# Roboy/gym-roboy

Hardware: AMD Instinct MI355X
Metric: env-steps/sec, MsjRobot (3-DOF/8-tendon) batched rollout (higher is better)
Workload: dtype f32

## Files before the change

### gym_roboy_amd/csrc/msj_kernels.hpp

```cpp
#pragma once
#include "rtc_compat.hpp"
#include "msj_math.hpp"
#include "philox.hpp"
#include "env_common.hpp"

#if defined(RB_JIT_TABLE)
namespace rbk { __device__ constexpr rb::MsjConst<float, 8> BAKED = RB_JIT_TABLE; }
#else
#include "msj_baked.hpp"
#endif

namespace rbk {

using rbe::EnvParams;
using rbe::GoalBox;
using rbe::goal_value;
using rbe::mul_then_add;

constexpr int NT8 = 8;
constexpr int RS = rb::MsjModel<float, 8>::RS;
using Const8 = rb::MsjConst<float, NT8>;
constexpr int NTX = 16;
using ConstX = rb::MsjConst<float, NTX>;

// ... 11 lines not shown

template <int KEEP>
struct SpSplit {
    const float *reg;
    const float *col;
    int stride;
    __device__ __forceinline__ float operator()(int k) const { return k < KEEP ? reg[k] : col[(k - KEEP) * stride]; }
};

struct Scale8 { float v[NT8]; };

template <int INTEG, int BLOCK, int UNROLL, bool BK = false>
__global__ void __launch_bounds__(BLOCK)
msj_step_env_per_lane(const Const8 c_arg, float *__restrict__ q, float *__restrict__ qd,
                      uint32_t *__restrict__ feas, const float *__restrict__ act, const Scale8 us, long n, long cnt) {
    const Const8 &c = robot_consts<BK>(c_arg);
    const long i = long(blockIdx.x) * BLOCK + threadIdx.x;
    if (i >= cnt) return;
    float qq[3], vv[3], sp[NT8];
    const float4 a0 = reinterpret_cast<const float4 *>(act)[2 * i];
    const float4 a1 = reinterpret_cast<const float4 *>(act)[2 * i + 1];
#pragma unroll
    for (int j = 0; j < 3; ++j) { qq[j] = q[j * n + i]; vv[j] = qd[j * n + i]; }
    const float a[NT8] = {a0.x, a0.y, a0.z, a0.w, a1.x, a1.y, a1.z, a1.w};
#pragma unroll
    for (int k = 0; k < NT8; ++k) sp[k] = a[k] * us.v[k];
    bool ok;
    if (UNROLL >= NT8) {
        ok = rb::MsjModel<float, NT8>::template step_sp<INTEG, UNROLL>(c, qq, vv, rb::SpArray<float, NT8>{sp});
    } else {
        __shared__ float lds_sp[NT8][BLOCK];
#pragma unroll
        for (int k = 0; k < NT8; ++k) lds_sp[k][threadIdx.x] = sp[k];
        ok = rb::MsjModel<float, NT8>::template step_sp<INTEG, UNROLL>(c, qq, vv, SpLds{&lds_sp[0][threadIdx.x], BLOCK});
    }
#pragma unroll
    for (int j = 0; j < 3; ++j) { q[j * n + i] = qq[j]; qd[j * n + i] = vv[j]; }
    feas[i] = ok ? 1u : 0u;
}




__device__ __forceinline__ __amdgpu_buffer_rsrc_t wg_rsrc(const void *base, int bytes) {
    return __builtin_amdgcn_make_buffer_rsrc(const_cast<void *>(base), 0, bytes, 0x00020000);
}

template <int INTEG, int BLOCK, bool BK = false>
__global__ void __launch_bounds__(BLOCK)
msj_step_env_per_lane_rs(const Const8 c_arg, float *__restrict__ q, float *__restrict__ qd,
                         uint32_t *__restrict__ feas, const float *__restrict__ act, const Scale8 us, long n, long cnt) {
    const Const8 &c = robot_consts<BK>(c_arg);
    const long env0 = long(blockIdx.x) * BLOCK;
    const long left = cnt - env0;
    const int live = int(left < BLOCK ? left : BLOCK);
    const int le = int(threadIdx.x);
    if (le >= live) return;
    const int off = le * 4;
    float qq[3], vv[3], u[NT8];
    const __amdgpu_buffer_rsrc_t ra = wg_rsrc(act + env0 * NT8, live * NT8 * 4);
    typedef float f4 __attribute__((ext_vector_type(4)));
    const f4 a0 = __builtin_bit_cast(f4, __builtin_amdgcn_raw_buffer_load_b128(ra, off * NT8, 0, 0));
    const f4 a1 = __builtin_bit_cast(f4, __builtin_amdgcn_raw_buffer_load_b128(ra, off * NT8 + 16, 0, 0));
#pragma unroll
    for (int j = 0; j < 3; ++j) {
        qq[j] = __uint_as_float(__builtin_amdgcn_raw_buffer_load_b32(wg_rsrc(q + j * n + env0, live * 4), off, 0, 0));
        vv[j] = __uint_as_float(__builtin_amdgcn_raw_buffer_load_b32(wg_rsrc(qd + j * n + env0, live * 4), off, 0, 0));
    }
    const float a[NT8] = {a0.x, a0.y, a0.z, a0.w, a1.x, a1.y, a1.z, a1.w};
#pragma unroll
    for (int k = 0; k < NT8; ++k) u[k] = a[k] * us.v[k];
    constexpr int KEEP = NT8 - 2;
    __shared__ float lds_u[NT8 - KEEP][BLOCK];
#pragma unroll
    for (int k = KEEP; k < NT8; ++k) lds_u[k - KEEP][le] = u[k];
    const bool ok = rb::MsjModel<float, NT8>::template step_rs_paired<INTEG>(c, qq, vv, SpSplit<KEEP>{u, &lds_u[0][le], BLOCK});
#pragma unroll
    for (int j = 0; j < 3; ++j) {
        __builtin_amdgcn_raw_buffer_store_b32(__float_as_uint(qq[j]), wg_rsrc(q + j * n + env0, live * 4), off, 0, 0);
        __builtin_amdgcn_raw_buffer_store_b32(__float_as_uint(vv[j]), wg_rsrc(qd + j * n + env0, live * 4), off, 0, 0);
    }
    __builtin_amdgcn_raw_buffer_store_b32(ok ? 1u : 0u, wg_rsrc(feas + env0, live * 4), off, 0, 0);
}


struct PairMap { int a[4], d[4]; };
struct Scale4 { float v[4]; };

template <int CTRL>
__device__ __forceinline__ float rbk_dpp(float v) {
    return __int_as_float(__builtin_amdgcn_update_dpp(0, __float_as_int(v), CTRL, 0xF, 0xF, true));
}

template <int MIRROR>
struct AccelMirrorHalf {
    const Const8 &c;
    const float *u;
    __device__ __forceinline__ void operator()(const float q[3], const float qd[3], float qdd[3]) const {
        using M = rb::MsjModel<float, NT8>;
        const M::Frame f = M::frame(q, qd);
        float tx, ty, tz;
        M::half_torque(c, f, u, tx, ty, tz);
        M::template mirror_combine<MIRROR>(tx, ty, tz, rbk_dpp<0xB1>(tx), rbk_dpp<0xB1>(ty), rbk_dpp<0xB1>(tz));
        M::rigid_body(c, f, qd, tx, ty, tz, qdd);
    }
};

template <int INTEG, int BLOCK, int MIRROR, bool BK = false>
__global__ void __launch_bounds__(BLOCK)
msj_step_mirror_pairs(const Const8 c_arg, const PairMap pm, float *__restrict__ q, float *__restrict__ qd,
                      uint32_t *__restrict__ feas, const float *__restrict__ act, const Scale4 us, long n, long cnt) {
    const Const8 &c = robot_consts<BK>(c_arg);
    const long env0 = long(blockIdx.x) * (BLOCK / 2);
    const long left = cnt - env0;
    const int live = int(left < BLOCK / 2 ? left : BLOCK / 2);
    const int le = int(threadIdx.x >> 1);
    if (le >= live) return;
    const bool odd = (threadIdx.x & 1) != 0;
    const int off = le * 4, oddi = int(threadIdx.x & 1);
    float qq[3], vv[3], u[4];
    const __amdgpu_buffer_rsrc_t ra = wg_rsrc(act + env0 * NT8, live * NT8 * 4);
#pragma unroll
    for (int k = 0; k < 4; ++k) u[k] = __uint_as_float(__builtin_amdgcn_raw_buffer_load_b32(ra, off * NT8 + pm.a[k] + oddi * pm.d[k], 0, 0)) * us.v[k];
#pragma unroll
    for (int j = 0; j < 3; ++j) {
        qq[j] = __uint_as_float(__builtin_amdgcn_raw_buffer_load_b32(wg_rsrc(q + j * n + env0, live * 4), off, 0, 0));
        vv[j] = __uint_as_float(__builtin_amdgcn_raw_buffer_load_b32(wg_rsrc(qd + j * n + env0, live * 4), off, 0, 0));
    }
    constexpr int F0 = MIRROR == 0 ? 0 : 1, F1 = 2;
    const uint32_t flip = odd ? 0x80000000u : 0u;
    qq[F0] = __uint_as_float(__float_as_uint(qq[F0]) ^ flip); vv[F0] = __uint_as_float(__float_as_uint(vv[F0]) ^ flip);
    qq[F1] = __uint_as_float(__float_as_uint(qq[F1]) ^ flip); vv[F1] = __uint_as_float(__float_as_uint(vv[F1]) ^ flip);
    const bool ok = rb::MsjModel<float, NT8>::template integrate_acc<INTEG>(c, qq, vv, AccelMirrorHalf<MIRROR>{c, u});
    const int soff = odd ? 0x7fffff00 : le * 4;
#pragma unroll
    for (int j = 0; j < 3; ++j) {
        __builtin_amdgcn_raw_buffer_store_b32(__float_as_uint(qq[j]), wg_rsrc(q + j * n + env0, live * 4), soff, 0, 0);
        __builtin_amdgcn_raw_buffer_store_b32(__float_as_uint(vv[j]), wg_rsrc(qd + j * n + env0, live * 4), soff, 0, 0);
    }
    __builtin_amdgcn_raw_buffer_store_b32(ok ? 1u : 0u, wg_rsrc(feas + env0, live * 4), soff, 0, 0);
}


template <int INTEG, int BLOCK, int UNROLL, bool BK = false>
__global__ void __launch_bounds__(BLOCK)
msj_rollout_fused(const Const8 c_arg, float *__restrict__ q, float *__restrict__ qd, uint32_t *__restrict__ feas,
                  const float *__restrict__ act_ring, int ring, int n_steps, const Scale8 us, long n) {
    const Const8 &c = robot_consts<BK>(c_arg);
    const long i = long(blockIdx.x) * BLOCK + threadIdx.x;
    if (i >= n) return;
    float qq[3], vv[3];
#pragma unroll
    for (int j = 0; j < 3; ++j) { qq[j] = q[j * n + i]; vv[j] = qd[j * n + i]; }
    bool ok = true;
    const float4 *rec = reinterpret_cast<const float4 *>(act_ring) + 2 * i;
    float4 a0 = rec[0], a1 = rec[1];
    __shared__ float lds_sp[UNROLL >= NT8 ? 1 : NT8][BLOCK];
    int slab = 0;
    for (int t = 0; t < n_steps; ++t) {
        const float a[NT8] = {a0.x, a0.y, a0.z, a0.w, a1.x, a1.y, a1.z, a1.w};
        float sp[NT8];
#pragma unroll
        for (int k = 0; k < NT8; ++k) sp[k] = a[k] * us.v[k];
        if (t + 1 < n_steps) {
            slab = slab + 1 == ring ? 0 : slab + 1;
            const float4 *nx = rec + long(slab) * 2 * n;
// ... 244 lines not shown
```

### gym_roboy_amd/csrc/msj_math.hpp

```cpp
#pragma once
#include "rtc_compat.hpp"

#if defined(__HIPCC__)
#define RB_HD __host__ __device__ __forceinline__
#else
#define RB_HD inline
#endif


namespace rb {

template <typename T> struct Fast;
template <> struct Fast<double> {
    static RB_HD void sincos(double x, double &s, double &c) { s = ::sin(x); c = ::cos(x); }
    static RB_HD double exp(double x) { return ::exp(x); }
    static RB_HD double exp2(double x) { return ::exp2(x); }
    static RB_HD double rsqrt(double x) { return 1.0 / ::sqrt(x); }
    static RB_HD double rcp(double x) { return 1.0 / x; }
};
template <> struct Fast<float> {
    static RB_HD void sincos(float x, float &s, float &c) {
#if defined(__HIP_DEVICE_COMPILE__)
        s = __sinf(x); c = __cosf(x);
#else
// ... 412 lines not shown
            }
            rigid_body(c, f, qd, tx, ty, tz, qdd);
        }
    };

    struct Routing { T d2, mx, my, mz; };
    static RB_HD Routing routing(const Frame &f, const MsjTendon<T> &t) {
        const T ax = f.r00 * t.A[0] + f.r10 * t.A[1] + f.r20 * t.A[2];
        const T ay = f.r01 * t.A[0] + f.r11 * t.A[1] + f.r21 * t.A[2];
        const T az = f.r02 * t.A[0] + f.r12 * t.A[1] + f.r22 * t.A[2];
        Routing r;
        r.d2 = ax * t.B2[0] + (ay * t.B2[1] + (az * t.B2[2] + t.ab2));
        r.mx = ay * t.Bv[2] - az * t.Bv[1];
        r.my = az * t.Bv[0] - ax * t.Bv[2];
        r.mz = ax * t.Bv[1] - ay * t.Bv[0];
        return r;
    }
    struct Strain { T v, es, fl, pe; };
    static RB_HD Strain strain(const C &c, const Frame &f, const MsjTendon<T> &t, const Routing &r, T inv) {
        Strain s;
        s.v = (f.wx * r.mx + f.wy * r.my + f.wz * r.mz) * inv;
        s.es = (r.d2 * inv) * t.il0s + t.elcs;
        s.fl = Fast<T>::exp2(-(s.es * s.es));
        s.pe = Fast<T>::exp2(c.pe_k2s * s.es);
        return s;
    }
    struct Hill { T afn, rden; };
    static RB_HD Hill hill(const C &c, const Strain &s, T u) {
        const T act = tclamp(c.kps * s.es - u, T(0), T(1));
        const T vp = tmax(s.v, T(0)), p = tclamp(s.v + T(1), T(0), T(1));
        const T num = c.fv_c1l * vp + p;
        const T den = c.fv_c2l * vp + (c.fv_c2s * p + c.fv_k);
        Hill h;
        h.rden = Fast<T>::rcp(den);
        h.afn = (act * s.fl) * num;
        return h;
    }
    static RB_HD void torque(const C &c, const MsjTendon<T> &t, const Routing &r, T inv, const Strain &s, const Hill &h,
                             T &tx, T &ty, T &tz) {
        const T fpe = tmax(s.pe * c.inv_pe_den - c.inv_pe_den, T(0));
        const T Fs = (t.fmaxv * inv) * (h.afn * h.rden + fpe);
        tx -= Fs * r.mx; ty -= Fs * r.my; tz -= Fs * r.mz;
    }
    static RB_HD void pin() {
#if defined(__HIP_DEVICE_COMPILE__)
        __builtin_amdgcn_sched_barrier(0);
#endif
    }
    static RB_HD void tendon_pair(const C &c, const Frame &f, const MsjTendon<T> &ta, const MsjTendon<T> &tb, T ua, T ub,
                                  T &tx, T &ty, T &tz) {
        const Routing ra = routing(f, ta);
        pin();
        const T ia = Fast<T>::rsqrt(ra.d2);
        const Routing rb_ = routing(f, tb);
        pin();
        const T ib = Fast<T>::rsqrt(rb_.d2);
        const Strain sa = strain(c, f, ta, ra, ia);
        pin();
        const Hill ha = hill(c, sa, ua);
        const Strain sb = strain(c, f, tb, rb_, ib);
        pin();
        torque(c, ta, ra, ia, sa, ha, tx, ty, tz);
        const Hill hb = hill(c, sb, ub);
        pin();
        torque(c, tb, rb_, ib, sb, hb, tx, ty, tz);
        pin();
    }
    template <typename SP>
    struct AccelPaired {
        const C &c;
        const SP &sp;
        RB_HD void operator()(const T q[3], const T qd[3], T qdd[3]) const {
            static_assert(NT % 2 == 0, "tendons in pairs");
            const Frame f = frame(q, qd);
            T tx = T(0), ty = T(0), tz = T(0);
#pragma unroll
            for (int k = 0; k < NT; k += 2) {
                const T ua = sp(k), ub = sp(k + 1);
                tendon_pair(c, f, c.ten[k], c.ten[k + 1], ua, ub, tx, ty, tz);
            }
            rigid_body(c, f, qd, tx, ty, tz, qdd);
        }
    };
    static constexpr int RS = 9;
    template <int INTEG>
    static RB_HD bool step_rs(const C &c, T q[3], T qd[3], const T u[NT]) {
        return integrate_acc<INTEG>(c, q, qd, AccelPinned{c, u});
    }

    template <int INTEG, typename SP>
    static RB_HD bool step_rs_paired(const C &c, T q[3], T qd[3], const SP &sp) {
        return integrate_acc<INTEG>(c, q, qd, AccelPaired<SP>{c, sp});
    }

    template <int INTEG, int UNROLL, typename SP>
    static RB_HD bool step_sp(const C &c, T q[3], T qd[3], const SP &sp) {
        return integrate<INTEG>(c, q, qd, AccelAllTendons<UNROLL, SP>{c, sp});
    }

    template <int INTEG, int UNROLL = NT>
    static RB_HD bool step(const C &c, T q[3], T qd[3], const T sp[NT]) {
        T u[NT];
#pragma unroll
        for (int k = 0; k < NT; ++k) u[k] = prescale(c, k, sp[k]);
        const SpArray<T, NT> src{u};
        return step_sp<INTEG, UNROLL>(c, q, qd, src);
    }
};

}
```

### gym_roboy_amd/csrc/roboy_dispatch.hpp

```cpp

enum : int { CLS_BALL8 = RB_CLASS_BALL8, CLS_BALLX = RB_CLASS_BALLX, CLS_TREE = RB_CLASS_TREE };
enum : int { ENTRY_STEP = RB_ENTRY_STEP, ENTRY_ENV = RB_ENTRY_ENV_STEP, ENTRY_FUSED = RB_ENTRY_FUSED_ROLLOUT };
enum : int { SRC_KERNARG = RB_SPEC_NONE, SRC_TABLE = RB_SPEC_TABLE, SRC_JIT = RB_SPEC_JIT };
constexpr int F_LANE = RB_KERNEL_ENV_PER_LANE, F_OCTET = RB_KERNEL_TENDON_PER_LANE, F_WAVE = RB_KERNEL_ENV_PER_WAVE, F_SPLIT = RB_KERNEL_ENV_PER_LANE_SPLIT,
              F_PAIR = RB_KERNEL_LANE_PAIR, F_SPLIT2 = RB_KERNEL_ENV_PER_LANE_SPLIT2;

struct Key {
    int cls, entry, form, integ, block, src, variant;
    bool operator==(const Key &o) const {
        return cls == o.cls && entry == o.entry && form == o.form && integ == o.integ && block == o.block && src == o.src && variant == o.variant;
    }
};

struct Launch {
    long i0 = 0, cnt = 0;
    hipStream_t stream = nullptr;
    const float *act = nullptr;
    float act_scale = 1.0f;
    float *obs = nullptr, *reward = nullptr; uint32_t *done = nullptr;
    int ring = 0, n_steps = 0;
};
using Launcher = int (*)(rb_sim *, const Launch &);

struct Row {
    Key key;
    bool ranges;
    Launcher launch;
};

inline Scale8 scale8(const rb_sim *s, float act_scale) {
    Scale8 us;
    for (int k = 0; k < NT8; ++k) us.v[k] = act_scale * s->c8.ten[k].ksg;
    return us;
}
inline PairMap pair_map(const rb_sim *s) {
    PairMap pm;
    for (int k = 0; k < 4; ++k) { pm.a[k] = 4 * s->pair_half[k]; pm.d[k] = 4 * (s->pair_image[k] - s->pair_half[k]); }
    return pm;
}

template <int INTEG, int B, int U, bool BK>
int l_msj_step(rb_sim *s, const Launch &L) {
    const Scale8 us = scale8(s, L.act_scale);
    float *q = s->d_q + L.i0, *qd = s->d_qd + L.i0;
    uint32_t *feas = s->d_feas + L.i0;
    const float *act = L.act + size_t(L.i0) * NT8;
    if constexpr (U == RS)
        hipLaunchKernelGGL((msj_step_env_per_lane_rs<INTEG, B, BK>), dim3(blocks_for(L.cnt, B)), dim3(B), 0, L.stream, s->c8, q, qd, feas, act, us, s->n, L.cnt);
    else
        hipLaunchKernelGGL((msj_step_env_per_lane<INTEG, B, U, BK>), dim3(blocks_for(L.cnt, B)), dim3(B), 0, L.stream, s->c8, q, qd, feas, act, us, s->n, L.cnt);
    return RB_OK;
}
int l_msj_step_jit(rb_sim *s, const Launch &L) {
    Const8 c8 = s->c8;
    Scale8 us = scale8(s, L.act_scale);
    float *q = s->d_q + L.i0, *qd = s->d_qd + L.i0;
    uint32_t *feas = s->d_feas + L.i0;
    const float *act = L.act + size_t(L.i0) * NT8;
    long nn = s->n, cc = L.cnt;
    void *args[] = {&c8, &q, &qd, &feas, &act, &us, &nn, &cc};
    RB_HIP(hipModuleLaunchKernel(s->jit.step[s->integrator == RB_EULER ? 0 : 1], blocks_for(L.cnt, 256), 1, 1, 256, 1, 1, 0, L.stream, args, nullptr));
    return RB_OK;
}
template <int INTEG, int B>
int l_msj_step_nt(rb_sim *s, const Launch &L) {
    hipLaunchKernelGGL((msj_step_env_per_lane_nt<INTEG, B>), dim3(blocks_for(s->n, B)), dim3(B), 0, L.stream, s->cx, s->d_q, s->d_qd, s->d_feas, L.act, L.act_scale, s->n);
    return RB_OK;
}
template <int INTEG, int B, int M, bool BK>
int l_msj_step_pair(rb_sim *s, const Launch &L) {
    const PairMap pm = pair_map(s);
    Scale4 us4;
    for (int k = 0; k < 4; ++k) us4.v[k] = L.act_scale * s->c8.ten[s->pair_half[k]].ksg;
    hipLaunchKernelGGL((msj_step_mirror_pairs<INTEG, B, M, BK>), dim3(blocks_for(2 * L.cnt, B)), dim3(B), 0, L.stream, s->c8p, pm,
                       s->d_q + L.i0, s->d_qd + L.i0, s->d_feas + L.i0, L.act + size_t(L.i0) * NT8, us4, s->n, L.cnt);
    return RB_OK;
}
template <int INTEG>
int l_msj_step_octet(rb_sim *s, const Launch &L) {
    hipLaunchKernelGGL((msj_step_tendon_per_lane<INTEG>), dim3(blocks_for(s->n * NT8, 64)), dim3(64), 0, L.stream, s->c8, s->d_ten, s->d_q, s->d_qd,
                       s->d_feas, L.act, L.act_scale, s->n);
    return RB_OK;
}

template <int INTEG, int B, int U, bool BK>
int l_msj_fused(rb_sim *s, const Launch &L) {
    const Scale8 us = scale8(s, L.act_scale);
    hipLaunchKernelGGL((msj_rollout_fused<INTEG, B, U, BK>), dim3(blocks_for(s->n, B)), dim3(B), 0, L.stream, s->c8, s->d_q, s->d_qd, s->d_feas, L.act,
                       L.ring, L.n_steps, us, s->n);
    return RB_OK;
}
int l_msj_fused_jit(rb_sim *s, const Launch &L) {
    Const8 c8 = s->c8;
    Scale8 us = scale8(s, L.act_scale);
    long nn = s->n;
    const float *ring_ptr = L.act;
    int ring = L.ring, n_steps = L.n_steps;
    void *args[] = {&c8, &s->d_q, &s->d_qd, &s->d_feas, &ring_ptr, &ring, &n_steps, &us, &nn};
    RB_HIP(hipModuleLaunchKernel(s->jit.rollout[s->integrator == RB_EULER ? 0 : 1], blocks_for(s->n, 256), 1, 1, 256, 1, 1, 0, L.stream, args, nullptr));
    return RB_OK;
}

inline MsjEnvArgs msj_env_args(rb_sim *s, const Launch &L) {
    const long i0 = L.i0;
    MsjEnvArgs a;
    a.e = s->env;
    for (int j = 0; j < 3; ++j) { a.box_lo[j] = s->box.lo[j]; a.box_hi[j] = s->box.hi[j]; }
    a.q = s->d_q + i0; a.qd = s->d_qd + i0; a.feas = s->d_feas + i0; a.goal = s->d_goal + i0; a.step_num = s->d_step_num + i0;
    a.ep_ret = s->d_ep_ret + i0; a.goal_count = s->d_goal_count + i0; a.act = L.act + i0 * s->n_t;
    a.obs = L.obs + i0 * 9; a.reward = L.reward + i0; a.done = L.done + i0;
    a.ep_sum = s->d_ep_sum + i0; a.ep_cnt = s->d_ep_cnt + i0; a.infeas_n = s->d_infeas_n + i0;
    a.n = s->n; a.cnt = L.cnt; a.seed = s->seed; a.env0 = uint64_t(s->env0) + uint64_t(i0);
    return a;
}
template <int INTEG, int B, int U, bool BK>
int l_msj_env(rb_sim *s, const Launch &L) {
    hipLaunchKernelGGL((msj_env_step_kernel<INTEG, B, U, Const8, BK>), dim3(blocks_for(L.cnt, B)), dim3(B), 0, L.stream, s->c8, msj_env_args(s, L));
    return RB_OK;
}
template <int INTEG, int B>
int l_msj_env_nt(rb_sim *s, const Launch &L) {
    hipLaunchKernelGGL((msj_env_step_kernel<INTEG, B, 0, ConstX>), dim3(blocks_for(L.cnt, B)), dim3(B), 0, L.stream, s->cx, msj_env_args(s, L));
    return RB_OK;
}
int l_msj_env_jit(rb_sim *s, const Launch &L) {
    Const8 c8 = s->c8;
    MsjEnvArgs a = msj_env_args(s, L);
    void *args[] = {&c8, &a};
    RB_HIP(hipModuleLaunchKernel(s->jit.env[s->integrator == RB_EULER ? 0 : 1], blocks_for(L.cnt, 256), 1, 1, 256, 1, 1, 0, L.stream, args, nullptr));
    return RB_OK;
}
template <int INTEG, int B, int M, bool BK>
// ... 313 lines not shown
```

### gym_roboy_amd/csrc/roboy_sim.hip

```cpp
#include <hip/hip_runtime.h>

#include <cmath>
#include <cstdio>
#include <cstring>
#include <map>
#include <string>
#include <vector>

#include "../../include/roboy_sim.h"
#include "msj_build.hpp"
#include "msj_kernels.hpp"
#include "msj_jit.hpp"
#include "tree_aba.hpp"
#include "tree_lane_defs.hpp"
#define RBL_NS rbl_baked
#include "tree_lane_baked.hpp"
#include "tree_lane.hpp"
#undef RBL_NS
#define RBL_NS rbl_split_baked
#include "tree_lane_split_baked.hpp"
#include "tree_lane_split.hpp"
#undef RBL_NS
#include "tree_lane_jit.hpp"
#include "tree_lane_split2.hpp"
#include "tendon_state.hpp"
#include "env_params.hpp"
#include "env_obs.hpp"
#include "env_io.hpp"
#include "env_hist.hpp"
#include "env_critic.hpp"
#include "env_goal.hpp"
#include "env_shaping.hpp"
#include "env_push.hpp"

namespace {

thread_local std::string g_err;

int fail(int code, const std::string &msg) { g_err = msg; return code; }

#define RB_HIP(call)                                                                      \
    do {                                                                                  \
        hipError_t e_ = (call);                                                           \
        if (e_ != hipSuccess)                                                             \
            return fail(RB_EHIP, std::string(#call) + ": " + hipGetErrorString(e_));      \
    } while (0)

#ifndef RB_SMALL_BATCH
#define RB_SMALL_BATCH 65536
#endif
#ifndef RB_TENDON_LANE_BATCH_EULER
#define RB_TENDON_LANE_BATCH_EULER 8192
#endif
#ifndef RB_TENDON_LANE_BATCH_RK4
#define RB_TENDON_LANE_BATCH_RK4 16384
#endif
#ifndef RB_TENDON_LANE_BATCH_PAIR_EULER
#define RB_TENDON_LANE_BATCH_PAIR_EULER 4096
#endif
#ifndef RB_TENDON_LANE_BATCH_PAIR_RK4
#define RB_TENDON_LANE_BATCH_PAIR_RK4 12288
#endif
#ifndef RB_BIG_BLOCK_EULER
#define RB_BIG_BLOCK_EULER 256
#endif
#ifndef RB_BIG_UNROLL_EULER
#define RB_BIG_UNROLL_EULER 2
#endif
#ifndef RB_BIG_BLOCK_RK4
#define RB_BIG_BLOCK_RK4 256
#endif
#ifndef RB_BIG_UNROLL_RK4
#define RB_BIG_UNROLL_RK4 2
#endif
#ifndef RB_BAKED_UNROLL_EULER
#define RB_BAKED_UNROLL_EULER 8
#endif
#ifndef RB_BAKED_UNROLL_RK4
#define RB_BAKED_UNROLL_RK4 RS
#endif
#ifndef RB_TREE_JIT_BATCH
#define RB_TREE_JIT_BATCH 16384
#endif
#ifndef RB_TREE_LANE_MAX_LIVE
#define RB_TREE_LANE_MAX_LIVE 400
#endif
#ifndef RB_TREE_SPLIT_BATCH
#define RB_TREE_SPLIT_BATCH 16384
#endif
#ifndef RB_TREE_SPLIT2_BATCH
#define RB_TREE_SPLIT2_BATCH 32768
#endif
#ifndef RB_PAIR_SMALL_BATCH
#define RB_PAIR_SMALL_BATCH 65536
#endif
#ifndef RB_PAIR_BATCH_EULER
#define RB_PAIR_BATCH_EULER 16384
#endif
#ifndef RB_PAIR_BATCH_RK4
#define RB_PAIR_BATCH_RK4 32768
#endif
#ifndef RB_PAIR_ENV_BATCH_EULER
#define RB_PAIR_ENV_BATCH_EULER 24576
#endif
#ifndef RB_PAIR_ENV_BATCH_RK4
#define RB_PAIR_ENV_BATCH_RK4 32768
#endif
#ifndef RB_OCTET_ENV_BATCH_EULER
#define RB_OCTET_ENV_BATCH_EULER 8192
#endif
#ifndef RB_OCTET_ENV_BATCH_RK4
#define RB_OCTET_ENV_BATCH_RK4 8192
#endif
using namespace rbk;


template <int INTEG, int BLOCK>
__global__ void __launch_bounds__(BLOCK)
msj_step_env_per_lane_nt(const ConstX c, float *__restrict__ q, float *__restrict__ qd,
                         uint32_t *__restrict__ feas, const float *__restrict__ act, float act_scale, long n) {
    const long i = long(blockIdx.x) * BLOCK + threadIdx.x;
    if (i >= n) return;
    __shared__ float lds_sp[NTX][BLOCK];
    const int nt = c.nt;
    const float *row = act + i * nt;
    for (int k = 0; k < nt; ++k) lds_sp[k][threadIdx.x] = row[k] * (act_scale * c.ten[k].ksg);
    float qq[3], vv[3];
#pragma unroll
    for (int j = 0; j < 3; ++j) { qq[j] = q[j * n + i]; vv[j] = qd[j * n + i]; }
    const bool ok = rb::MsjModel<float, NTX>::template step_sp<INTEG, 0>(c, qq, vv, SpLds{&lds_sp[0][threadIdx.x], BLOCK});
#pragma unroll
    for (int j = 0; j < 3; ++j) { q[j * n + i] = qq[j]; qd[j * n + i] = vv[j]; }
    feas[i] = ok ? 1u : 0u;
}

template <int CTRL>
__device__ __forceinline__ float dpp_move(float v) {
    return __int_as_float(__builtin_amdgcn_update_dpp(0, __float_as_int(v), CTRL, 0xF, 0xF, true));
}
__device__ __forceinline__ float sum8(float v) {
    v += dpp_move<0xB1>(v);
    v += dpp_move<0x4E>(v);
    v += dpp_move<0x141>(v);
    return v;
}

struct AccelOneTendon {
    const Const8 &c;
    const rb::MsjTendon<float> &t;
    float spk;
    __device__ __forceinline__ void operator()(const float q[3], const float qd[3], float qdd[3]) const {
        using M = rb::MsjModel<float, NT8>;
        const M::Frame f = M::frame(q, qd);
        float tx = 0.0f, ty = 0.0f, tz = 0.0f;
        M::tendon(c, f, t, spk, tx, ty, tz);
        tx = sum8(tx); ty = sum8(ty); tz = sum8(tz);
        M::rigid_body(c, f, qd, tx, ty, tz, qdd);
    }
};

__device__ __forceinline__ unsigned xcd_block() {
    const unsigned nb = gridDim.x, xcd = blockIdx.x & 7u, qn = nb >> 3, rn = nb & 7u;
// ... 187 lines not shown
    goal_count[i] = draw + 1u;
    for (int j = 0; j < 3; ++j) {
        q[j * n + i] = 0.0f; qd[j * n + i] = 0.0f; goal[j * n + i] = g[j];
        if (obs) { obs[i * 9 + j] = 0.0f; obs[i * 9 + 3 + j] = 0.0f; obs[i * 9 + 6 + j] = g[j]; }
    }
    feas[i] = 1u; step_num[i] = 1u; ep_ret[i] = 0.0f;
}

inline unsigned blocks_for(long n, int block) { return unsigned((n + block - 1) / block); }

struct OptParams {
    bool on = false, resample = false; int n = 0;
    float *d_planes = nullptr, *d_ranges = nullptr; uint32_t *d_draws = nullptr;
    std::vector<float> ranges;
    void release() { (void)hipFree(d_planes); (void)hipFree(d_draws); (void)hipFree(d_ranges); *this = OptParams{}; }
    int need() const { return on ? RB_OK : fail(RB_EINVAL, "per-env parameters are not enabled (rb_params_enable)"); }
};
struct OptChannels { int mask = 0; float scale[4] = {1.0f, 1.0f, 1.0f, 1.0f}; void release() { *this = OptChannels{}; } };
struct OptIo {
    bool on = false; rb_env_io_config cfg = {};
    uint32_t *d_delay = nullptr, *d_draws = nullptr, *d_rows = nullptr;
    float *d_ring = nullptr; int slots = 0;
    void release() { (void)hipFree(d_delay); (void)hipFree(d_draws); (void)hipFree(d_rows); (void)hipFree(d_ring); *this = OptIo{}; }
};
struct OptActionRows { int rows = 0; void release() { rows = 0; } };
struct OptDoneKind {
    bool on = false; uint32_t *d_seen = nullptr, *d_kind = nullptr;
    void release() { (void)hipFree(d_seen); (void)hipFree(d_kind); *this = OptDoneKind{}; }
    int need() const { return on ? RB_OK : fail(RB_EINVAL, "episode-end codes are not enabled (rb_env_done_kind_configure)"); }
};
struct OptCritic {
    int mask = 0, dim = 0; float *d_rows = nullptr;
    void release() { (void)hipFree(d_rows); *this = OptCritic{}; }
    int need() const { return mask ? RB_OK : fail(RB_EINVAL, "critic rows are not enabled (rb_env_critic_obs_configure)"); }
};
struct OptGoals {
    float *d_pool = nullptr; int64_t m = 0;
    uint32_t L = 0, up = 0, down = 0;
    uint32_t *d_level = nullptr, *d_index = nullptr, *d_seen = nullptr;
    uint64_t *d_hist = nullptr, *d_row_stats = nullptr;
    void release() { (void)hipFree(d_pool); (void)hipFree(d_level); (void)hipFree(d_row_stats); *this = OptGoals{}; }
    int need_pool() const { return d_pool ? RB_OK : fail(RB_EINVAL, "no goal pool is set (rb_env_goal_pool_set)"); }
    int need_curriculum() const { return L ? RB_OK : fail(RB_EINVAL, "no goal curriculum is configured (rb_env_goal_curriculum_configure)"); }
    int need_row_stats() const { return d_row_stats ? RB_OK : fail(RB_EINVAL, "goal row stats are not enabled (rb_env_goal_row_stats_enable)"); }
};
struct OptShaping {
    bool on = false; rb_env_shaping_config cfg = {};
    float *d_prev = nullptr, *d_cost = nullptr;
    double *d_run = nullptr, *d_sums = nullptr, *d_red = nullptr; uint32_t *d_cnt = nullptr;
    int tree_waves = 1;
    bool tendons() const { return on && (cfg.tension != 0.0f || cfg.activation != 0.0f); }
    void release() {
        (void)hipFree(d_prev); (void)hipFree(d_cost); (void)hipFree(d_run); (void)hipFree(d_sums); (void)hipFree(d_red); (void)hipFree(d_cnt);
        *this = OptShaping{};
    }
    int need() const { return on ? RB_OK : fail(RB_EINVAL, "reward shaping is not configured (rb_env_shaping_configure)"); }
};
struct OptPush {
    bool on = false; rb_env_push_config cfg = {};
    uint32_t *d_count = nullptr, *d_last = nullptr, *d_n = nullptr;
    float *d_impulse = nullptr; unsigned long long *d_total = nullptr;
    void release() {
        (void)hipFree(d_count); (void)hipFree(d_last); (void)hipFree(d_n); (void)hipFree(d_impulse); (void)hipFree(d_total);
        *this = OptPush{};
    }
    int need() const { return on ? RB_OK : fail(RB_EINVAL, "random pushes are not configured (rb_env_push_configure)"); }
};

}

struct rb_sim {
    int device = 0, n_cu = 256;
    long n = 0;
    int n_q = 0, n_t = 0;
    int integrator = 0, nsub = 1, kernel = RB_KERNEL_ENV_PER_LANE;
    double step_size = 0.1;
    uint64_t seed = 0;
    int64_t env0 = 0;
    Const8 c8;
    ConstX cx;
    bool ntx = false;
    bool baked = false;
    int jit_state = 0;
    rbj::Module jit;
    std::string jit_why;
    rb::MsjTendon<float> *d_ten = nullptr;
    bool pair_ok = false, pair_baked = false;
    int pair_mirror = 0;
    int pair_half[4] = {0, 1, 2, 3}, pair_image[4] = {7, 6, 5, 4};
    Const8 c8p;
    int kernel_choice = RB_KERNEL_AUTO;
    bool tree = false;
    rbt::TreeHost tree_host;
    uint32_t *d_tree_words = nullptr;
    int tree_waves = 1;
    rblj::TreeForm forms[rblg::N_FORMS];
    static int form_index(int kernel) {
        return kernel == RB_KERNEL_ENV_PER_LANE_SPLIT ? rblg::FORM_SPLIT : kernel == RB_KERNEL_ENV_PER_LANE_SPLIT2 ? rblg::FORM_SPLIT2 : rblg::FORM_LANE;
    }
    rblj::TreeForm &form(int kernel) { return forms[form_index(kernel)]; }
    const rblj::TreeForm &form(int kernel) const { return forms[form_index(kernel)]; }
    GoalBox box;
    hipStream_t own_stream = nullptr, stream = nullptr;
    static constexpr int MAX_CHAINS = 4;
    int chains_choice = 0;
    hipStream_t chain_stream[MAX_CHAINS] = {};
    hipEvent_t chain_fork = nullptr, chain_join[MAX_CHAINS] = {};
    static constexpr int MAX_CALLER_STREAMS = 8;
    struct CallerStream { hipStream_t stream = nullptr; hipEvent_t done = nullptr; bool pending = false; uint64_t tick = 0; };
    CallerStream caller[MAX_CALLER_STREAMS];
    uint64_t caller_tick = 0;
    hipStream_t call_stream = nullptr;
    float *d_q = nullptr, *d_qd = nullptr;
    uint32_t *d_feas = nullptr, *d_goal_count = nullptr;
    bool env_ready = false;
    EnvParams env;
    float *d_goal = nullptr, *d_ep_ret = nullptr;
    double *d_ep_sum = nullptr;
    uint32_t *d_ep_cnt = nullptr;
    uint32_t *d_step_num = nullptr, *d_infeas_n = nullptr;
    double *d_stats = nullptr;
    double env_steps = 0.0;
    float *d_rows = nullptr;
    float *d_state_rows = nullptr, *h_state_rows = nullptr;
    uint8_t *d_u8 = nullptr;
    struct GraphKey {
        const float *ring_ptr; int ring; int chunk; float scale; int kernel;
        bool operator<(const GraphKey &o) const {
            return std::memcmp(this, &o, sizeof(GraphKey)) < 0;
        }
    };
    struct ChainGraphs {
        hipGraphExec_t exec[MAX_CHAINS] = {};
        int chains = 1;
        void destroy() { for (hipGraphExec_t &e : exec) { if (e) (void)hipGraphExecDestroy(e); e = nullptr; } }
    };
    std::map<GraphKey, ChainGraphs> graphs;
    rbts::Units<rbk::NTX> ts_units;
    std::vector<float> ts_tree_lconst;
    float *d_ts_lconst = nullptr, *d_ts_out = nullptr;
    bool ts_attr_set = false;
    OptParams par; OptChannels chan; OptIo io; OptActionRows hist; OptDoneKind done; OptCritic critic; OptGoals goals;
    OptShaping shaping;
    OptPush push;
    float qd_max[32] = {};
    int obs_dim() const { return 3 * n_q + rbo::n_channels(chan.mask) * n_t + hist.rows * n_t; }
    int critic_width() const { return rbc::row_dim(critic.mask, n_q, par.on ? par.n : 0, hist.rows * n_t); }
};

namespace {

bool stream_capturing(hipStream_t stream) {
    hipStreamCaptureStatus st = hipStreamCaptureStatusNone;
    return stream && hipStreamIsCapturing(stream, &st) == hipSuccess && st != hipStreamCaptureStatusNone;
}
bool capturing(rb_sim *s) { return stream_capturing(s->stream) || (s->call_stream && stream_capturing(s->call_stream)); }
struct CallStreamScope {
    rb_sim *s;
    CallStreamScope(rb_sim *sim, hipStream_t st) : s(sim) { s->call_stream = st; }
    ~CallStreamScope() { s->call_stream = nullptr; }
};

int jit_level() {
    const char *e = std::getenv("ROBOY_SIM_JIT");
    return e && e[0] >= '0' && e[0] <= '2' ? e[0] - '0' : 1;
}
// ... 119 lines not shown
    if (s->own_stream && s->own_stream != s->stream) RB_HIP(hipStreamSynchronize(s->own_stream));
    for (int c = 1; c < rb_sim::MAX_CHAINS; ++c)
        if (s->chain_stream[c]) RB_HIP(hipStreamSynchronize(s->chain_stream[c]));
    for (rb_sim::CallerStream &c : s->caller)
        if (c.pending) { RB_HIP(hipEventSynchronize(c.done)); c.pending = false; }
    return RB_OK;
}
int note_caller_stream(rb_sim *s, hipStream_t st) {
    if (st == s->stream || st == s->own_stream) return RB_OK;
    for (int c = 1; c < rb_sim::MAX_CHAINS; ++c) if (st == s->chain_stream[c] && st) return RB_OK;
    if (stream_capturing(st)) return RB_OK;
    rb_sim::CallerStream *slot = nullptr;
    for (rb_sim::CallerStream &c : s->caller) if (c.done && c.stream == st) { slot = &c; break; }
    if (!slot) {
        for (rb_sim::CallerStream &c : s->caller) if (!c.done) { slot = &c; break; }
        if (!slot) {
            slot = &s->caller[0];
            for (rb_sim::CallerStream &c : s->caller) if (c.tick < slot->tick) slot = &c;
            if (slot->pending) { RB_HIP(hipEventSynchronize(slot->done)); slot->pending = false; }
        } else {
            RB_HIP(hipEventCreateWithFlags(&slot->done, chain_event_flags()));
        }
        slot->stream = st;
    }
    RB_HIP(hipEventRecord(slot->done, st));
    slot->pending = true;
    slot->tick = ++s->caller_tick;
    return RB_OK;
}
int drop_graphs(rb_sim *s) {
    if (s->graphs.empty()) return RB_OK;
    int rc = drain(s);
    if (rc) return rc;
    for (auto &kv : s->graphs) kv.second.destroy();
    s->graphs.clear();
    return RB_OK;
}

int range_ok(const rb_sim *s, int64_t first, int64_t count) {
    if (first < 0 || count < 1 || first + count > s->n) return fail(RB_EINVAL, "range outside the batch");
    if (first % 256) return fail(RB_EINVAL, "a range starts at a multiple of 256 envs");
    return RB_OK;
}

}

#include "env_host.hpp"

extern "C" {

const char *rb_last_error(void) { return g_err.c_str(); }
int rb_abi_version(void) { return RB_ABI_VERSION; }

int rb_device_count(int *count) {
    if (!count) return fail(RB_EINVAL, "count is null");
    *count = 0;
    RB_HIP(hipGetDeviceCount(count));
    return RB_OK;
}

int rb_create(const rb_robot_desc *robot, int64_t n_envs, int integrator, double step_size,
              int n_substeps, int device, uint64_t seed, int64_t env_id_offset, rb_sim **out) {
    if (!robot || !out) return fail(RB_EINVAL, "robot/out is null");
    *out = nullptr;
    if (n_envs < 1) return fail(RB_EINVAL, "n_envs must be >= 1");
    if (integrator != RB_EULER && integrator != RB_RK4) return fail(RB_EINVAL, "unknown integrator");
    if (!(step_size > 0.0) || n_substeps < 1) return fail(RB_EINVAL, "step_size must be > 0 and n_substeps >= 1");
    if (robot->n_q < 1 || robot->n_q > 32 || robot->n_t < 1) return fail(RB_EINVAL, "n_q must be in [1, 32], n_t >= 1");
    if (n_envs > (int64_t(1) << 30)) return fail(RB_EINVAL, "n_envs too large");
    if (env_id_offset < 0) return fail(RB_EINVAL, "env_id_offset must be >= 0");

    rb_sim *s = new (std::nothrow) rb_sim();
    if (!s) return fail(RB_ENOMEM, "out of host memory");
    std::string why;
    int rc = rb::msj_build<float, NT8>(robot, step_size, n_substeps, &s->c8, why);
    if (rc == RB_OK) {
        const Const8 &a = s->c8, &b = rbk::BAKED_HOST;
        auto same = [](const float *x, const float *y, int n) { return std::memcmp(x, y, sizeof(float) * size_t(n)) == 0; };
        bool eq = same(a.IO, b.IO, 6) && same(a.mc, b.mc, 3) && same(a.g, b.g, 3) && same(a.arm, b.arm, 3) && same(a.damp, b.damp, 3) &&
                  same(a.qlo, b.qlo, 3) && same(a.qhi, b.qhi, 3) && same(a.qdmax, b.qdmax, 3) && same(&a.kps, &b.kps, 8) &&
                  a.nsub == b.nsub && a.simple == b.simple && a.nt == b.nt;
        for (int k = 0; k < NT8 && eq; ++k) eq = same(a.ten[k].A, b.ten[k].A, 16);
        s->baked = eq;
        s->pair_ok = rb::find_mirror_pairs(s->c8, s->pair_mirror, s->pair_half, s->pair_image);
        if (s->pair_ok) {
            s->c8p = s->c8;
            bool first_four = true;
            for (int k = 0; k < 4; ++k) { s->c8p.ten[k] = s->c8.ten[s->pair_half[k]]; first_four = first_four && s->pair_half[k] == k; }
            s->pair_baked = s->baked && first_four;
        }
    }
    if (rc == RB_EUNSUPPORTED && robot->n_t != NT8) {
        std::string why_x;
        if (rb::msj_build<float, NTX>(robot, step_size, n_substeps, &s->cx, why_x, false) == RB_OK) {
            s->ntx = true;
            rc = RB_OK;
        }
    }
    if (rc == RB_EUNSUPPORTED) {
        std::string why_tree;
        rc = rbt::tree_build(robot, step_size, n_substeps, s->tree_host, why_tree);
        if (rc == RB_OK) {
            s->tree = true;
            for (int f = 0; f < rblg::N_FORMS; ++f) {
                std::string why_gen;
                s->forms[f].ok = (f != rblg::FORM_SPLIT2 || s->forms[rblg::FORM_SPLIT].ok) &&
                                 rblg::generate_form(robot, f, s->forms[f].gen, why_gen) == RB_OK;
            }
            rblj::TreeForm &lane = s->forms[rblg::FORM_LANE], &split = s->forms[rblg::FORM_SPLIT], &split2 = s->forms[rblg::FORM_SPLIT2];
            lane.baked = lane.ok && lane.gen.hash == RBL_TEXT_HASH && lane.gen.lds == size_t(rbl_baked::LDS_BYTES_PER_WAVE);
            split.baked = split.ok && split.gen.hash == RBL_SPLIT_TEXT_HASH && split.gen.n_parts == RBL_NPARTS &&
                          split.gen.n_helpers == RBL_NHELPERS && split.gen.lds == size_t(rbl_split_baked::SP_LDS_BYTES);
            split2.baked = split2.ok && robot->n_q == rbs2::n_q() && robot->n_t == rbs2::n_t() && split2.gen.hash == rbs2::text_hash() &&
                           split2.gen.n_parts == rbs2::n_parts() && split2.gen.lds == rbs2::lds_bytes();
        }
        else why = "not a ball-joint robot (" + why + ") and not a supported joint tree (" + why_tree + ")";
    }
    if (rc != RB_OK) {
        delete s;
        return fail(rc, "no HIP kernel for this robot structure: " + why);
    }
    if (s->tree) rbt::tree_tendon_lconst(robot, s->ts_tree_lconst);
    else rb::msj_tendon_units(robot, s->ts_units.u, NTX);
    int count = 0;
    hipError_t e = hipGetDeviceCount(&count);
    if (e != hipSuccess || count < 1) {
        delete s;
        return fail(RB_EHIP, std::string("no HIP device available: ") + hipGetErrorString(e));
    }
    if (device < 0 || device >= count) { delete s; return fail(RB_EINVAL, "device index out of range"); }
    s->device = device; s->n = n_envs; s->n_q = robot->n_q; s->n_t = robot->n_t;
    s->integrator = integrator; s->nsub = n_substeps; s->step_size = step_size;
    s->seed = seed; s->env0 = env_id_offset;
    for (int j = 0; j < s->n_q; ++j) { s->box.lo[j] = float(robot->q_lo[j]); s->box.hi[j] = float(robot->q_hi[j]); s->qd_max[j] = float(robot->qd_max[j]); }

#define RB_TRY(call)                                                                      \
    do {                                                                                  \
        hipError_t e_ = (call);                                                           \
        if (e_ != hipSuccess) {                                                           \
            std::string m_ = std::string(#call) + ": " + hipGetErrorString(e_);           \
            rb_destroy(s);                                                                \
            return fail(e_ == hipErrorOutOfMemory ? RB_ENOMEM : RB_EHIP, m_);             \
        }                                                                                 \
    } while (0)
    RB_TRY(hipSetDevice(device));
    {
        hipDeviceProp_t prop;
        RB_TRY(hipGetDeviceProperties(&prop, device));
        s->n_cu = prop.multiProcessorCount > 0 ? prop.multiProcessorCount : 256;
    }
    RB_TRY(hipStreamCreateWithFlags(&s->own_stream, hipStreamNonBlocking));
    s->stream = s->own_stream;
    const size_t plane = sizeof(float) * size_t(n_envs);
    RB_TRY(hipMalloc(&s->d_q, plane * s->n_q));
    RB_TRY(hipMalloc(&s->d_qd, plane * s->n_q));
    RB_TRY(hipMalloc(&s->d_feas, sizeof(uint32_t) * size_t(n_envs)));
    RB_TRY(hipMalloc(&s->d_goal_count, sizeof(uint32_t) * size_t(n_envs)));
    const int width = s->n_q > s->n_t ? s->n_q : s->n_t;
    RB_TRY(hipMalloc(&s->d_rows, plane * width));
    RB_TRY(hipMalloc(&s->d_u8, size_t(n_envs)));
    RB_TRY(hipMalloc(&s->d_state_rows, plane * (2 * s->n_q + 1)));
    RB_TRY(hipHostMalloc(reinterpret_cast<void **>(&s->h_state_rows), plane * (2 * s->n_q + 1), hipHostMallocDefault));
    if (!s->tree) {
        RB_TRY(hipMalloc(&s->d_ten, sizeof(s->c8.ten)));
        RB_TRY(hipMemcpyAsync(s->d_ten, s->c8.ten, sizeof(s->c8.ten), hipMemcpyHostToDevice, s->stream));
    } else {
// ... 633 lines not shown
```

Baseline: 20.26 billion.

## Add packed-fp32 two-tendon muscle kernel for baked RK4 env-per-lane step

Adds a new per-lane step kernel that evaluates tendon pairs with 2-wide float vectors (packed FMA) for the routing, strain, Hill and torque stages, interleaving two pairs at a time. The aim is to cut VALU instruction count through packed fp32 math on CDNA. It is dispatched for baked constants, INTEG==1, block 256 and batches up to a threshold, and can be turned off with an environment variable. Transcendentals stay scalar, and the extra vector packing and select ops could offset the gains or raise register pressure.

Result: slower. 19.67 billion (-2.9%).

```diff
diff --git a/gym_roboy_amd/csrc/msj_kernels.hpp b/gym_roboy_amd/csrc/msj_kernels.hpp
--- a/gym_roboy_amd/csrc/msj_kernels.hpp
+++ b/gym_roboy_amd/csrc/msj_kernels.hpp
@@ -117,6 +117,41 @@
     }
     __builtin_amdgcn_raw_buffer_store_b32(ok ? 1u : 0u, wg_rsrc(feas + env0, live * 4), off, 0, 0);
 }
+
+#if !defined(RB_JIT_TABLE)
+template <int BLOCK>
+__global__ void __launch_bounds__(BLOCK)
+msj_step_env_per_lane_pk(const Const8 c_arg, float *__restrict__ q, float *__restrict__ qd,
+                         uint32_t *__restrict__ feas, const float *__restrict__ act, const Scale8 us, long n, long cnt) {
+    const Const8 &c = robot_consts<true>(c_arg);
+    const long env0 = long(blockIdx.x) * BLOCK;
+    const long left = cnt - env0;
+    const int live = int(left < BLOCK ? left : BLOCK);
+    const int le = int(threadIdx.x);
+    if (le >= live) return;
+    const int off = le * 4;
+    float qq[3], vv[3], u[NT8];
+    const __amdgpu_buffer_rsrc_t ra = wg_rsrc(act + env0 * NT8, live * NT8 * 4);
+    typedef float f4 __attribute__((ext_vector_type(4)));
+    const f4 a0 = __builtin_bit_cast(f4, __builtin_amdgcn_raw_buffer_load_b128(ra, off * NT8, 0, 0));
+    const f4 a1 = __builtin_bit_cast(f4, __builtin_amdgcn_raw_buffer_load_b128(ra, off * NT8 + 16, 0, 0));
+#pragma unroll
+    for (int j = 0; j < 3; ++j) {
+        qq[j] = __uint_as_float(__builtin_amdgcn_raw_buffer_load_b32(wg_rsrc(q + j * n + env0, live * 4), off, 0, 0));
+        vv[j] = __uint_as_float(__builtin_amdgcn_raw_buffer_load_b32(wg_rsrc(qd + j * n + env0, live * 4), off, 0, 0));
+    }
+    const float a[NT8] = {a0.x, a0.y, a0.z, a0.w, a1.x, a1.y, a1.z, a1.w};
+#pragma unroll
+    for (int k = 0; k < NT8; ++k) u[k] = a[k] * us.v[k];
+    const bool ok = rb::MsjModel<float, NT8>::template step_rs_packed<1>(c, qq, vv, u);
+#pragma unroll
+    for (int j = 0; j < 3; ++j) {
+        __builtin_amdgcn_raw_buffer_store_b32(__float_as_uint(qq[j]), wg_rsrc(q + j * n + env0, live * 4), off, 0, 0);
+        __builtin_amdgcn_raw_buffer_store_b32(__float_as_uint(vv[j]), wg_rsrc(qd + j * n + env0, live * 4), off, 0, 0);
+    }
+    __builtin_amdgcn_raw_buffer_store_b32(ok ? 1u : 0u, wg_rsrc(feas + env0, live * 4), off, 0, 0);
+}
+#endif
 
 
 struct PairMap { int a[4], d[4]; };
diff --git a/gym_roboy_amd/csrc/msj_math.hpp b/gym_roboy_amd/csrc/msj_math.hpp
--- a/gym_roboy_amd/csrc/msj_math.hpp
+++ b/gym_roboy_amd/csrc/msj_math.hpp
@@ -518,6 +518,104 @@
             rigid_body(c, f, qd, tx, ty, tz, qdd);
         }
     };
+#if defined(__HIPCC__)
+    typedef float f2 __attribute__((ext_vector_type(2)));
+    static __device__ __forceinline__ f2 pk_fma(f2 a, f2 b, f2 c) { return __builtin_elementwise_fma(a, b, c); }
+    static __device__ __forceinline__ f2 pair_of(float a, float b) { f2 r; r.x = a; r.y = b; return r; }
+    static __device__ __forceinline__ f2 both(float a) { f2 r; r.x = a; r.y = a; return r; }
+#define RB_PK(m) pair_of(ta.m, tb.m)
+    struct PkRouting { f2 d2, mx, my, mz; };
+    static __device__ __forceinline__ PkRouting pk_routing(const Frame &f, const MsjTendon<T> &ta, const MsjTendon<T> &tb) {
+#pragma clang fp contract(off)
+        static_assert(std::is_same<T, float>::value, "packed pairs are fp32");
+        const f2 ax = pk_fma(both(f.r20), RB_PK(A[2]), pk_fma(both(f.r00), RB_PK(A[0]), both(f.r10) * RB_PK(A[1])));
+        const f2 ay = pk_fma(both(f.r21), RB_PK(A[2]), pk_fma(both(f.r01), RB_PK(A[0]), both(f.r11) * RB_PK(A[1])));
+        const f2 az = pk_fma(both(f.r22), RB_PK(A[2]), pk_fma(both(f.r02), RB_PK(A[0]), both(f.r12) * RB_PK(A[1])));
+        PkRouting r;
+        r.d2 = pk_fma(ax, RB_PK(B2[0]), pk_fma(ay, RB_PK(B2[1]), pk_fma(az, RB_PK(B2[2]), RB_PK(ab2))));
+        const f2 mx_n = pk_fma(ay, RB_PK(Bv[2]), -(az * RB_PK(Bv[1]))), mx_r = pk_fma(-az, RB_PK(Bv[1]), ay * RB_PK(Bv[2]));
+        const f2 mz_n = pk_fma(ax, RB_PK(Bv[1]), -(ay * RB_PK(Bv[0]))), mz_r = pk_fma(-ay, RB_PK(Bv[0]), ax * RB_PK(Bv[1]));
+        const bool rxa = ta.Bv[1] < 0.0f, rxb = tb.Bv[1] < 0.0f, rza = rxa && ta.Bv[0] < 0.0f, rzb = rxb && tb.Bv[0] < 0.0f;
+        r.mx = pair_of(rxa ? mx_r.x : mx_n.x, rxb ? mx_r.y : mx_n.y);
+        r.my = pk_fma(az, RB_PK(Bv[0]), -(ax * RB_PK(Bv[2])));
+        r.mz = pair_of(rza ? mz_r.x : mz_n.x, rzb ? mz_r.y : mz_n.y);
+        return r;
+    }
+    static __device__ __forceinline__ f2 pk_rsqrt(f2 d2) { return pair_of(Fast<float>::rsqrt(d2.x), Fast<float>::rsqrt(d2.y)); }
+    struct PkStrain { f2 dot, v, es, fl, pe; };
+    static __device__ __forceinline__ PkStrain pk_strain(const C &c, const Frame &f, const MsjTendon<T> &ta, const MsjTendon<T> &tb,
+                                                         const PkRouting &r, f2 inv) {
+#pragma clang fp contract(off)
+        PkStrain s;
+        s.dot = pk_fma(both(f.wz), r.mz, pk_fma(both(f.wx), r.mx, both(f.wy) * r.my));
+        s.v = s.dot * inv;
+        s.es = pk_fma(r.d2 * inv, RB_PK(il0s), RB_PK(elcs));
+        const f2 fla = -(s.es * s.es), pea = both(c.pe_k2s) * s.es;
+        s.fl = pair_of(Fast<float>::exp2(fla.x), Fast<float>::exp2(fla.y));
+        s.pe = pair_of(Fast<float>::exp2(pea.x), Fast<float>::exp2(pea.y));
+        return s;
+    }
+    struct PkHill { f2 act, num, rden; };
+    static __device__ __forceinline__ PkHill pk_hill(const C &c, const PkStrain &s, f2 inv, float ua, float ub) {
+#pragma clang fp contract(off)
+        PkHill h;
+        h.act = pair_of(tclamp(__builtin_fmaf(s.es.x, c.kps, -ua), 0.0f, 1.0f), tclamp(__builtin_fmaf(s.es.y, c.kps, -ub), 0.0f, 1.0f));
+        const f2 vp = pair_of(tmax(s.v.x, 0.0f), tmax(s.v.y, 0.0f));
+        const f2 p = pair_of(tclamp(__builtin_fmaf(s.dot.x, inv.x, 1.0f), 0.0f, 1.0f), tclamp(__builtin_fmaf(s.dot.y, inv.y, 1.0f), 0.0f, 1.0f));
+        h.num = pk_fma(both(c.fv_c1l), vp, p);
+        const f2 den = pk_fma(both(c.fv_c2l), vp, pk_fma(both(c.fv_c2s), p, both(c.fv_k)));
+        h.rden = pair_of(Fast<float>::rcp(den.x), Fast<float>::rcp(den.y));
+        return h;
+    }
+    static __device__ __forceinline__ void pk_torque(const C &c, const MsjTendon<T> &ta, const MsjTendon<T> &tb, const PkRouting &r, f2 inv,
+                                                     const PkStrain &s, const PkHill &h, float &tx, float &ty, float &tz) {
+#pragma clang fp contract(off)
+        const f2 fpa = pk_fma(s.pe, both(c.inv_pe_den), both(-c.inv_pe_den));
+        const f2 fpe = pair_of(tmax(fpa.x, 0.0f), tmax(fpa.y, 0.0f));
+        const f2 Fs = (RB_PK(fmaxv) * inv) * pk_fma((h.act * s.fl) * h.num, h.rden, fpe);
+        tx = __builtin_fmaf(-r.mx.x, Fs.x, tx); ty = __builtin_fmaf(-r.my.x, Fs.x, ty); tz = __builtin_fmaf(-r.mz.x, Fs.x, tz);
+        tx = __builtin_fmaf(-r.mx.y, Fs.y, tx); ty = __builtin_fmaf(-r.my.y, Fs.y, ty); tz = __builtin_fmaf(-r.mz.y, Fs.y, tz);
+    }
+#undef RB_PK
+    static __device__ __forceinline__ void tendon_quad_packed(const C &c, const Frame &f, const MsjTendon<T> &ta, const MsjTendon<T> &tb,
+                                                              const MsjTendon<T> &tc, const MsjTendon<T> &td, float ua, float ub, float uc,
+                                                              float ud, float &tx, float &ty, float &tz) {
+        const PkRouting rp = pk_routing(f, ta, tb);
+        pin();
+        const f2 ip = pk_rsqrt(rp.d2);
+        const PkRouting rq = pk_routing(f, tc, td);
+        pin();
+        const f2 iq = pk_rsqrt(rq.d2);
+        const PkStrain sp = pk_strain(c, f, ta, tb, rp, ip);
+        pin();
+        const PkHill hp = pk_hill(c, sp, ip, ua, ub);
+        const PkStrain sq = pk_strain(c, f, tc, td, rq, iq);
+        pin();
+        pk_torque(c, ta, tb, rp, ip, sp, hp, tx, ty, tz);
+        const PkHill hq = pk_hill(c, sq, iq, uc, ud);
+        pin();
+        pk_torque(c, tc, td, rq, iq, sq, hq, tx, ty, tz);
+        pin();
+    }
+    struct AccelPacked {
+        const C &c;
+        const float *u;
+        __device__ __forceinline__ void operator()(const T q[3], const T qd[3], T qdd[3]) const {
+            static_assert(NT % 4 == 0, "tendons in pairs of pairs");
+            const Frame f = frame(q, qd);
+            T tx = T(0), ty = T(0), tz = T(0);
+#pragma unroll
+            for (int k = 0; k < NT; k += 4)
+                tendon_quad_packed(c, f, c.ten[k], c.ten[k + 1], c.ten[k + 2], c.ten[k + 3], u[k], u[k + 1], u[k + 2], u[k + 3], tx, ty, tz);
+            rigid_body(c, f, qd, tx, ty, tz, qdd);
+        }
+    };
+    template <int INTEG>
+    static __device__ __forceinline__ bool step_rs_packed(const C &c, T q[3], T qd[3], const T u[NT]) {
+        return integrate_acc<INTEG>(c, q, qd, AccelPacked{c, u});
+    }
+#endif
+
     static constexpr int RS = 9;
     template <int INTEG>
     static RB_HD bool step_rs(const C &c, T q[3], T qd[3], const T u[NT]) {
diff --git a/gym_roboy_amd/csrc/roboy_dispatch.hpp b/gym_roboy_amd/csrc/roboy_dispatch.hpp
--- a/gym_roboy_amd/csrc/roboy_dispatch.hpp
+++ b/gym_roboy_amd/csrc/roboy_dispatch.hpp
@@ -45,9 +45,15 @@
     float *q = s->d_q + L.i0, *qd = s->d_qd + L.i0;
     uint32_t *feas = s->d_feas + L.i0;
     const float *act = L.act + size_t(L.i0) * NT8;
-    if constexpr (U == RS)
+    if constexpr (U == RS) {
+        if constexpr (BK && INTEG == 1 && B == 256) {
+            if (s->packed && s->n <= RB_PACKED_MAX_BATCH) {
+                hipLaunchKernelGGL((msj_step_env_per_lane_pk<B>), dim3(blocks_for(L.cnt, B)), dim3(B), 0, L.stream, s->c8, q, qd, feas, act, us, s->n, L.cnt);
+                return RB_OK;
+            }
+        }
         hipLaunchKernelGGL((msj_step_env_per_lane_rs<INTEG, B, BK>), dim3(blocks_for(L.cnt, B)), dim3(B), 0, L.stream, s->c8, q, qd, feas, act, us, s->n, L.cnt);
-    else
+    } else
         hipLaunchKernelGGL((msj_step_env_per_lane<INTEG, B, U, BK>), dim3(blocks_for(L.cnt, B)), dim3(B), 0, L.stream, s->c8, q, qd, feas, act, us, s->n, L.cnt);
     return RB_OK;
 }
diff --git a/gym_roboy_amd/csrc/roboy_sim.hip b/gym_roboy_amd/csrc/roboy_sim.hip
--- a/gym_roboy_amd/csrc/roboy_sim.hip
+++ b/gym_roboy_amd/csrc/roboy_sim.hip
@@ -78,6 +78,9 @@
 #endif
 #ifndef RB_BAKED_UNROLL_RK4
 #define RB_BAKED_UNROLL_RK4 RS
+#endif
+#ifndef RB_PACKED_MAX_BATCH
+#define RB_PACKED_MAX_BATCH 393216
 #endif
 #ifndef RB_TREE_JIT_BATCH
 #define RB_TREE_JIT_BATCH 16384
@@ -431,6 +434,7 @@
     bool ntx = false;
     bool baked = false;
     int jit_state = 0;
+    bool packed = true;
     rbj::Module jit;
     std::string jit_why;
     rb::MsjTendon<float> *d_ten = nullptr;
@@ -716,6 +720,7 @@
                   a.nsub == b.nsub && a.simple == b.simple && a.nt == b.nt;
         for (int k = 0; k < NT8 && eq; ++k) eq = same(a.ten[k].A, b.ten[k].A, 16);
         s->baked = eq;
+        if (const char *e = std::getenv("ROBOY_SIM_PACKED")) s->packed = e[0] != '0';
         s->pair_ok = rb::find_mirror_pairs(s->c8, s->pair_mirror, s->pair_half, s->pair_image);
         if (s->pair_ok) {
             s->c8p = s->c8;
```
